# chao-ji/ldm_tf2

Measured on AMD Instinct MI355X. Metric: images/sec (256x256, 200 DDIM steps, CFG=5), higher is better.
Workload: dtype bf16

## Files before the change

### ldm_tf2_amd/csrc/gemm.hip

```cpp
#include "gemm_kernel.h"
#include "gemm3_kernel.h"

using namespace ldm_gemm_detail;

namespace {

__global__ __launch_bounds__(256) void splitk_epilogue_kernel(GemmArgs p) {
  const int nout = p.act == LDM_ACT_GEGLU ? p.N / 2 : p.N;
  const int64_t total = (int64_t)p.M * nout;
  for (int64_t idx = (int64_t)blockIdx.x * 256 + threadIdx.x; idx < total;
       idx += (int64_t)gridDim.x * 256) {
    const int m = (int)(idx / nout), c = (int)(idx - (int64_t)m * nout);
    if (p.act == LDM_ACT_GEGLU) {
      const int nv = (c >> 5) * 64 + (c & 31), ng = nv + 32;
      float a = 0.f, g = 0.f;
      for (int s = 0; s < p.split_k; ++s) {
        const float* ws = p.ws + ((int64_t)s * p.M + m) * p.N;
        a += ws[nv]; g += ws[ng];
      }
      epi_store(p, 0, m, c, epi_pre(p, m, nv, a) * gelu_erf_f(epi_pre(p, m, ng, g)));
    } else {
      float a = 0.f;
      for (int s = 0; s < p.split_k; ++s) a += p.ws[((int64_t)s * p.M + m) * p.N + c];
      epi_store(p, 0, m, c, apply_act(p.act, epi_pre(p, m, c, a)));
// ... 23 lines not shown
    const f32x4 t0 = *(const f32x4*)(src + s * slab), t1 = *(const f32x4*)(src + s * slab + 4);
#pragma unroll
    for (int e = 0; e < 4; ++e) { v[e] += t0[e]; v[4 + e] += t1[e]; }
  }
  if (p.bias) {
    const f32x4 b0 = *(const f32x4*)(p.bias + nlog), b1 = *(const f32x4*)(p.bias + nlog + 4);
#pragma unroll
    for (int e = 0; e < 4; ++e) { v[e] = v[e] * p.alpha + b0[e]; v[4 + e] = v[4 + e] * p.alpha + b1[e]; }
  } else {
#pragma unroll
    for (int e = 0; e < 8; ++e) v[e] *= p.alpha;
  }
  if (p.addend) {
    const float* ad = p.addend + (int64_t)(m / p.add_rows) * p.add_ld + nlog;
    const f32x4 a0 = *(const f32x4*)ad, a1 = *(const f32x4*)(ad + 4);
#pragma unroll
    for (int e = 0; e < 4; ++e) { v[e] += a0[e]; v[4 + e] += a1[e]; }
  }
}

__global__ __launch_bounds__(256) void splitk_epilogue_vec_kernel(GemmArgs p) {
  const bool geglu = p.act == LDM_ACT_GEGLU;
  const int nout = geglu ? p.N / 2 : p.N;
  const int pcols = nout / 8;
  const int64_t total = (int64_t)p.M * pcols;
  for (int64_t idx = (int64_t)blockIdx.x * 256 + threadIdx.x; idx < total;
       idx += (int64_t)gridDim.x * 256) {
    const int m = (int)(idx / pcols), c = (int)(idx - (int64_t)m * pcols) * 8;
    const int nlog = geglu ? (c >> 5) * 64 + (c & 31) : c;
    float v[8];
    splitk_sum8(p, m, nlog, v);
    if (geglu) {
      float g[8];
      splitk_sum8(p, m, nlog + 32, g);
#pragma unroll
      for (int e = 0; e < 8; ++e) v[e] *= gelu_erf_f(g[e]);
    } else if (p.act != LDM_ACT_NONE) {
#pragma unroll
      for (int e = 0; e < 8; ++e) v[e] = apply_act(p.act, v[e]);
    }
    const int64_t ooff = (int64_t)m * p.ldc_m + c;
    const int64_t roff = (int64_t)m * p.ldr + c;
    if (p.out_dtype == LDM_BF16) {
      if (p.residual) {
        float rr[8];
        chunk_to_f32(*(const u32x4*)((const bf16_t*)p.residual + roff), rr, bf16_t());
#pragma unroll
        for (int e = 0; e < 8; ++e) v[e] += rr[e];
      }
      *(u32x4*)((bf16_t*)p.out + ooff) = f32_to_chunk(v, bf16_t());
    } else {
      if (p.residual) {
        const f32x4 r0 = *(const f32x4*)((const float*)p.residual + roff);
        const f32x4 r1 = *(const f32x4*)((const float*)p.residual + roff + 4);
#pragma unroll
        for (int e = 0; e < 4; ++e) { v[e] += r0[e]; v[4 + e] += r1[e]; }
      }
      f32x4 o0 = {v[0], v[1], v[2], v[3]}, o1 = {v[4], v[5], v[6], v[7]};
      *(f32x4*)((float*)p.out + ooff) = o0;
      *(f32x4*)((float*)p.out + ooff + 4) = o1;
    }
  }
}

struct TileCfg { int bm, bn; };
constexpr int kNumTiles = 20;
constexpr TileCfg kTiles[kNumTiles] = {{0, 0}, {256, 128}, {128, 128}, {128, 64}, {64, 64}, {256, 128},
                                       {128, 160}, {256, 160}, {128, 320},
                                       {256, 160}, {128, 160}, {256, 128}, {128, 128},
                                       {256, 160}, {256, 128},
                                       {256, 160}, {256, 128},
                                       {64, 64}, {128, 64}, {128, 128}};
constexpr int kResident[kNumTiles] = {0, 1, 2, 3, 5, 1, 2, 1, 1, 1, 2, 1, 2, 1, 1, 1, 1, 2, 2, 1};
constexpr bool kBf16Only[kNumTiles] = {false, false, false, false, false, false, false, false, false, true, true, true, true, true, true,
                                       true, true, false, false, false};
constexpr bool is_persistent(int c) { return c == 13 || c == 14; }
constexpr bool is_halo_ring(int c) { return c == 15 || c == 16; }
bool halo_ring_ok(const ldm_gemm_params* p) {
  return p->conv && p->stride == 1 && !p->upsample && !p->no_lead_pad && p->dtype == LDM_BF16 && p->batch == 1 &&
         (p->W == 16 || p->W == 32) && 256 % p->W == 0 && p->H % (256 / p->W) == 0 && p->M % 256 == 0 &&
         p->OH == p->H && p->OW == p->W;
}

template <typename T>
void launch_mode(int cfg, const GemmArgs& a, dim3 grid, hipStream_t s) {
  if (cfg == 15 || cfg == 16) {
    if constexpr (sizeof(T) == 2) launch_cfg<T, 3>(cfg, a, grid, s);
    return;
  }
  if (!a.conv) launch_cfg<T, 0>(cfg, a, grid, s);
  else if (!a.upsample) launch_cfg<T, 1>(cfg, a, grid, s);
  else launch_cfg<T, 2>(cfg, a, grid, s);
}

inline int cdiv(int a, int b) { return (a + b - 1) / b; }

void choose(const ldm_gemm_params* p, int esize, int* cfg_out, int* split_out) {
  static const double kStepUs[kNumTiles] = {0, 0.82, 0.82, 0.75, 0.87, 0.82, 1.12, 1.18, 1.15, 1.03, 1.09, 0.97, 0.80, 1.03, 0.97, 1.0, 0.94, 0.87, 0.75, 0.82};
  static const double kOverheadSteps[kNumTiles] = {0, 8, 8, 7, 6, 8, 8, 8, 8, 8, 8, 8, 8, 4, 4, 9, 9, 6, 7, 8};
  static const int kSplits[] = {1, 2, 3, 4, 5, 6, 8, 10, 12, 16, 20, 24, 32};
#ifdef LDM_TOOLS_BUILD
  static const bool no160 = getenv("LDM_GEMM_NO160") != nullptr;
  static const bool no_t2pref = getenv("LDM_GEMM_NO_T2PREF") != nullptr;
#else
  constexpr bool no160 = false, no_t2pref = false;
#endif
  const int bke = 128 / esize;
  const int ktiles = cdiv(p->K, bke);
  const bool geglu = p->act == LDM_ACT_GEGLU;
  const double f32x = esize == 4 ? 8.0 : 1.0;
  double best = 1e30;
  int best_cfg = 2, best_split = 1;
  for (int c = 1; c < kNumTiles; ++c) {
    if (p->tile > 0 && p->tile < kNumTiles && c != p->tile) continue;
    if (c == 5 && p->tile != 5) continue;
    if (c >= 13 && p->tile != c) continue;
    if (c == 12 && p->tile != c) continue;
    if ((c == 1 || c == 7) && esize == 2 && p->tile != c) continue;
    if (c == 6 && esize == 2 && p->tile != 6) continue;
    if (kBf16Only[c] && esize != 2) continue;
    if (p->a2 && (is_persistent(c) || is_halo_ring(c)) && p->tile != c) continue;
    if (kTiles[c].bn % 160 == 0 && p->tile != c && (p->N % kTiles[c].bn != 0 || no160)) continue;
    if (p->out2 && p->n_split % kTiles[c].bn != 0) continue;
    if (geglu && c > 2 && c != 5 && c != 11 && c != 12 && c != 14 && c != 19) continue;
    const TileCfg t = kTiles[c];
    const double tiles = (double)cdiv(p->M, t.bm) * cdiv(p->N, t.bn) * p->batch;
    for (int split : kSplits) {
      if (p->split_k > 0 && split != p->split_k) continue;
      if (is_persistent(c) && split > 1) continue;
      if (split > 1 && (p->batch != 1 || ktiles / split < 4 || tiles >= 256.0 * kResident[c] ||
                        (p->split_k <= 0 && (!p->workspace || (size_t)split * p->M * p->N * 4 > p->workspace_bytes))))
        continue;
      const int kps = cdiv(ktiles, split);
      const double rounds = (double)(int64_t)((tiles * split + 256.0 * kResident[c] - 1) / (256.0 * kResident[c]));
      double us = rounds * (kps + kOverheadSteps[c]) * kStepUs[c] * f32x;
      if (!no_t2pref && c == 2 && (double)cdiv(p->M, 256) * cdiv(p->N, 128) * p->batch < 256.0) us *= 0.9;
      if (split > 1) us += 3.0 + (double)p->M * p->N * 4.0 * (split + 1) / 3.0e6;
      if (us < best) { best = us; best_cfg = c; best_split = split; }
    }
  }
  if (p->split_k > 0 && p->batch == 1) best_split = p->split_k;
  if (p->tile > 0 && p->tile < kNumTiles) best_cfg = p->tile;
  else if (best_cfg == 9 && halo_ring_ok(p) && p->N % 160 == 0 && !p->out2 && !p->ln_out && !p->a2 && ktiles / best_split >= 27)
    best_cfg = 15;
  *cfg_out = best_cfg;
  *split_out = best_split;
}

void final_plan(const ldm_gemm_params* p, int* cfg_out, int* split_out, int* kps_out) {
  const int esize = p->dtype == LDM_BF16 ? 2 : 4;
  int cfg, split;
  choose(p, esize, &cfg, &split);
  if (p->ln_out) { cfg = kLnTile; split = 1; }
  if (p->ln_cs && !is_persistent(cfg)) {
    cfg = (p->act == LDM_ACT_GEGLU || p->N % 160 != 0) ? 14 : (p->N % 128 == 0 && p->tile != 13 ? 14 : 13);
    split = 1;
  }
  if (p->out2 && !is_persistent(cfg)) split = 1;
  if (is_persistent(cfg)) split = 1;
  const int ktiles = cdiv(p->K, 128 / esize);
  int kps = cdiv(ktiles, split < 1 ? 1 : split);
  if (is_halo_ring(cfg)) kps = cdiv(kps, 9) * 9;
  split = cdiv(ktiles, kps);
  *cfg_out = cfg; *split_out = split; *kps_out = kps;
}

void build_args(const ldm_gemm_params* p, int cfg, int split, int kps, GemmArgs* out) {
  const int esize = p->dtype == LDM_BF16 ? 2 : 4;
  const int bke = 128 / esize;
  int64_t a_bytes;
  if (p->conv) a_bytes = (((int64_t)p->B * p->H * p->W - 1) * p->lda + p->Cin) * esize;
  else a_bytes = (((int64_t)p->M - 1) * p->lda + (p->K - (p->a2 ? p->Cin2 : 0))) * esize;
  const int64_t w_bytes = (int64_t)p->N * p->K * esize;
  GemmArgs a;
  memset(&a, 0, sizeof(a));
  a.a = (const char*)p->a; a.w = (const char*)p->w; a.bias = p->bias; a.addend = p->addend;
  a.residual = (const char*)p->residual; a.out = (char*)p->out; a.ws = (float*)p->workspace;
  a.lda = p->lda; a.ldr = p->ldr; a.ldc_m = p->ldc_m; a.ldc_n = p->ldc_n;
  a.stride_a = p->stride_a; a.stride_w = p->stride_w; a.stride_c = p->stride_c; a.stride_r = p->stride_r;
  a.add_ld = p->add_ld; a.M = p->M; a.N = p->N; a.K = p->K; a.batch = p->batch;
  a.a_bytes = (uint32_t)a_bytes; a.w_bytes = (uint32_t)w_bytes;
  a.add_rows = p->add_rows > 0 ? p->add_rows : 1;
  a.conv = p->conv; a.H = p->H; a.W = p->W; a.Cin = p->Cin; a.OH = p->OH; a.OW = p->OW;
  a.stride = p->stride; a.upsample = p->upsample; a.pad = p->no_lead_pad ? 0 : 1; a.act = p->act; a.out_dtype = p->out_dtype;
  a.alpha = p->alpha;
  a.ln_out = (char*)p->ln_out; a.ln_gamma = p->ln_gamma; a.ln_beta = p->ln_beta; a.ld_ln = p->ld_ln;
  a.ln_eps = p->ln_eps;
  a.out2 = (char*)p->out2; a.ld2 = p->ld2; a.stride2 = p->stride2; a.n_split = p->n_split; a.rows2 = p->rows2;
  a.kt9 = cdiv(p->K, bke);
  if (p->a2) {
    a.a2 = (const char*)p->a2; a.lda2 = p->lda2; a.kt9 = (p->K - p->Cin2) / bke;
    a.a2_bytes = (uint32_t)((((int64_t)p->M - 1) * p->lda2 + p->Cin2) * esize);
  }
  const int nout = p->act == LDM_ACT_GEGLU ? p->N / 2 : p->N;
  auto al = [](const void* q, int by) { return ((uintptr_t)q % by) == 0; };
  a.vec_epilogue =
      p->ldc_n == 1 && nout % 8 == 0 && p->ldc_m % 8 == 0 && p->stride_c % 8 == 0 && al(p->out, 16) &&
      (!p->residual || (p->ldr % 8 == 0 && p->stride_r % 8 == 0 && al(p->residual, 16))) &&
      (!p->bias || al(p->bias, 16)) &&
      (!p->addend || (al(p->addend, 16) && p->add_ld % 4 == 0));
  a.ktiles = cdiv(p->K, bke);
  a.split_k = split;
  a.ktiles_per_split = kps;
  const TileCfg t = kTiles[cfg];
  a.tiles_m = cdiv(p->M, t.bm);
  a.tiles_n = cdiv(p->N, t.bn);
  *out = a;
}

int launch_reduce(const ldm_gemm_params* p, const GemmArgs& a, hipStream_t s) {
  const int nout = p->act == LDM_ACT_GEGLU ? p->N / 2 : p->N;
  const bool vec = a.vec_epilogue && ((uintptr_t)p->workspace % 16) == 0 && p->N % 4 == 0;
  int64_t total = vec ? (int64_t)p->M * (nout / 8) : (int64_t)p->M * nout;
  int blocks = (int)((total + 255) / 256);
  if (blocks > 4096) blocks = 4096;
  if (vec) hipLaunchKernelGGL(splitk_epilogue_vec_kernel, dim3(blocks), dim3(256), 0, s, a);
  else hipLaunchKernelGGL(splitk_epilogue_kernel, dim3(blocks), dim3(256), 0, s, a);
  return ldm_launch_status("ldm_gemm(splitk epilogue)");
}

}

extern "C" int ldm_gemm_splits(const ldm_gemm_params* p) {
  if (!p || !(p->dtype == LDM_F32 || p->dtype == LDM_BF16) || p->K <= 0) return 0;
  int cfg, split, kps;
  final_plan(p, &cfg, &split, &kps);
  return split;
}

extern "C" int ldm_gemm_reduce(const ldm_gemm_params* p, void* stream) {
  LDM_CHECK_ARG(p && p->out && p->workspace, "ldm_gemm_reduce: null pointer");
  int cfg, split, kps;
  final_plan(p, &cfg, &split, &kps);
  LDM_CHECK_ARG(split > 1, "ldm_gemm_reduce: these parameters do not split K (nothing was deferred)");
  LDM_CHECK_ARG(p->workspace_bytes >= (size_t)split * p->M * p->N * 4, "ldm_gemm_reduce: workspace too small");
  GemmArgs a;
  build_args(p, cfg, split, kps, &a);
  return launch_reduce(p, a, (hipStream_t)stream);
}

extern "C" size_t ldm_gemm_workspace_bytes(const ldm_gemm_params* p) {
  if (!p) return 0;
  int cfg, split, kps;
  final_plan(p, &cfg, &split, &kps);
  return split > 1 ? (size_t)split * p->M * p->N * 4 : 0;
}

extern "C" int ldm_gemm_ln_supported(int N, int dtype) {
  return (N == kTiles[kLnTile].bn && (dtype == LDM_F32 || dtype == LDM_BF16)) ? 1 : 0;
}

extern "C" int ldm_gemm_plan(const ldm_gemm_params* p, int* tile, int* split_k) {
  LDM_CHECK_ARG(p && tile && split_k, "ldm_gemm_plan: null pointer");
  LDM_CHECK_ARG(p->dtype == LDM_F32 || p->dtype == LDM_BF16, "ldm_gemm_plan: bad dtype %d", p->dtype);
  int kps;
  final_plan(p, tile, split_k, &kps);
  return LDM_OK;
}

extern "C" int ldm_gemm(const ldm_gemm_params* p, void* stream) {
  LDM_CHECK_ARG(p && p->a && p->w && p->out, "ldm_gemm: null pointer");
  LDM_CHECK_ARG(p->dtype == LDM_F32 || p->dtype == LDM_BF16, "ldm_gemm: bad dtype %d", p->dtype);
  LDM_CHECK_ARG(p->out_dtype == LDM_F32 || p->out_dtype == LDM_BF16, "ldm_gemm: bad out_dtype");
  LDM_CHECK_ARG(p->M > 0 && p->N > 0 && p->K > 0 && p->batch > 0, "ldm_gemm: bad M/N/K/batch");
  const int esize = p->dtype == LDM_BF16 ? 2 : 4;
  const int osize = p->out_dtype == LDM_BF16 ? 2 : 4;
  const int epc = 16 / esize, bke = 8 * epc;
  LDM_CHECK_ARG(p->K % bke == 0, "ldm_gemm: K=%d must be a multiple of the K-tile (%d elements)", p->K, bke);
  LDM_CHECK_ARG(((uintptr_t)p->a % 16) == 0 && ((uintptr_t)p->w % 16) == 0,
                "ldm_gemm: a/w must be 16-byte aligned");
  LDM_CHECK_ARG(p->lda % epc == 0 && p->stride_a % epc == 0 && p->stride_w % epc == 0,
                "ldm_gemm: lda/stride_a/stride_w must be multiples of %d elements", epc);
  int64_t a_bytes;
  if (p->conv) {
    LDM_CHECK_ARG(p->Cin > 0 && p->Cin % bke == 0, "ldm_gemm(conv): Cin=%d must be a multiple of %d",
                  p->Cin, bke);
    LDM_CHECK_ARG(p->K == 9 * p->Cin + (p->a2 ? p->Cin2 : 0), "ldm_gemm(conv): K must be 9*Cin (+ Cin2 with a second operand)");
    if (p->a2) {
      LDM_CHECK_ARG(p->stride == 1 && !p->upsample && !p->no_lead_pad && p->OH == p->H && p->OW == p->W,
                    "ldm_gemm(conv): the second operand (a2) needs a stride-1, pad-1, non-upsampled convolution");
      LDM_CHECK_ARG(p->Cin2 > 0 && p->Cin2 % bke == 0 && p->lda2 % epc == 0 && p->lda2 >= p->Cin2 && ((uintptr_t)p->a2 % 16) == 0,
                    "ldm_gemm(conv): a2 needs Cin2 %% %d == 0, lda2 %% %d == 0 and 16-byte alignment", bke, epc);
      LDM_CHECK_ARG((((int64_t)p->M - 1) * p->lda2 + p->Cin2) * esize < (1ll << 31), "ldm_gemm(conv): a2 extent must be < 2 GiB");
    }
    LDM_CHECK_ARG(p->stride == 1 || p->stride == 2, "ldm_gemm(conv): stride must be 1 or 2");
    LDM_CHECK_ARG(p->B > 0 && p->H > 0 && p->W > 0 && p->OH > 0 && p->OW > 0, "ldm_gemm(conv): dims");
    LDM_CHECK_ARG(p->H < 32768 && p->W < 32768, "ldm_gemm(conv): H/W too large");
    LDM_CHECK_ARG(!(p->upsample && p->stride != 1), "ldm_gemm(conv): upsample needs stride 1");
    const int hs = p->upsample ? 2 * p->H : p->H, wsz = p->upsample ? 2 * p->W : p->W;
    LDM_CHECK_ARG(!p->no_lead_pad || p->stride == 2, "ldm_gemm(conv): no_lead_pad needs stride 2");
    const int padsum = p->no_lead_pad ? 1 : 2;
    LDM_CHECK_ARG(p->OH == (hs + padsum - 3) / p->stride + 1 && p->OW == (wsz + padsum - 3) / p->stride + 1,
                  "ldm_gemm(conv): OH/OW inconsistent with H/W/stride/upsample");
    LDM_CHECK_ARG(p->M == p->B * p->OH * p->OW, "ldm_gemm(conv): M != B*OH*OW");
    LDM_CHECK_ARG(p->batch == 1, "ldm_gemm(conv): batch must be 1");
    a_bytes = (((int64_t)p->B * p->H * p->W - 1) * p->lda + p->Cin) * esize;
  } else {
    a_bytes = (((int64_t)p->M - 1) * p->lda + p->K) * esize;
  }
  const int64_t w_bytes = (int64_t)p->N * p->K * esize;
  LDM_CHECK_ARG(a_bytes < (1ll << 31) && w_bytes < (1ll << 31),
                "ldm_gemm: operand extent must be < 2 GiB (a=%lld w=%lld bytes)", (long long)a_bytes,
                (long long)w_bytes);
  if (p->addend) LDM_CHECK_ARG(p->add_rows > 0, "ldm_gemm: add_rows must be > 0 with addend");
// ... 35 lines not shown
  if (p->act == LDM_ACT_GEGLU) LDM_CHECK_ARG(cfg <= 2 || cfg == 5 || cfg == 11 || cfg == 12 || cfg == 14 || cfg == 19, "ldm_gemm: GEGLU needs a tile whose width is a multiple of 64 (1, 2, 5, 11, 12)");
  LDM_CHECK_ARG(!kBf16Only[cfg] || esize == 2, "ldm_gemm: tile %d is bf16 only", cfg);
  LDM_CHECK_ARG(!p->a2 || (!is_persistent(cfg) && !is_halo_ring(cfg) && cfg < kNumTiles),
                "ldm_gemm: tile %d cannot take a second A operand (a2): implicit-GEMM tiles 1-12, 17-19 only", cfg);
  if (is_halo_ring(cfg))
    LDM_CHECK_ARG(halo_ring_ok(p) && p->N % kTiles[cfg].bn == 0 && !p->out2 && !p->ln_out,
                  "ldm_gemm: tile %d (halo-staged conv) needs a bf16 stride-1 3x3 convolution with W = 16 or 32, "
                  "H %% (256 / W) == 0, M %% 256 == 0 and N %% %d == 0", cfg, kTiles[cfg].bn);
  if (is_persistent(cfg)) {
    const int bn = kTiles[cfg].bn;
    auto al16 = [](const void* q) { return ((uintptr_t)q % 16) == 0; };
    const bool trans = p->out2 != nullptr;
    const bool ln = p->ln_cs != nullptr;
    const bool nsplit_out = trans && p->n_split > 0;
    if (ln)
      LDM_CHECK_ARG(!p->conv && p->bias && al16(p->ln_cs) && p->ln_eps > 0.f && !p->addend && !p->residual,
                    "ldm_gemm: ln_cs (LayerNorm fold) needs plain rows, the folded bias, ln_eps > 0 and no addend / residual");
    if (trans)
      LDM_CHECK_ARG((p->n_split == 0 || (ln && p->n_split % bn == 0 && p->n_split < p->N)) && !p->conv && (!p->bias || ln) &&
                        !p->addend && !p->residual && p->act == LDM_ACT_NONE &&
                        p->rows2 > 0 && p->rows2 % 32 == 0 && p->M % p->rows2 == 0 && p->ld2 % 8 == 0 && p->stride2 % 8 == 0 &&
                        al16(p->out2),
                    "ldm_gemm: tile %d transposed output needs n_split 0 (or, LayerNorm-folded, whole n-tiles below it), a plain "
                    "product, rows2 %% 32 == 0, ld2 / stride2 %% 8 == 0", cfg);
    LDM_CHECK_ARG(p->dtype == LDM_BF16 && p->out_dtype == LDM_BF16 && p->batch == 1 && p->ldc_n == 1 &&
                      !p->ln_out && split <= 1 && p->N % bn == 0 && ((trans && !nsplit_out) || (p->ldc_m % 8 == 0 && al16(p->out))) &&
                      (!p->residual || (p->ldr % 4 == 0 && al16(p->residual))) && (!p->bias || al16(p->bias)) &&
                      (!p->addend || (al16(p->addend) && p->add_ld % 4 == 0)),
                  "ldm_gemm: tile %d (persistent) needs bf16 in/out, batch 1, a row-major 16-byte-aligned output, "
                  "N %% %d == 0, no split-K / out2 / ln_out", cfg, bn);
    Gemm3Args g;
    memset(&g, 0, sizeof(g));
    g.a = (const char*)p->a; g.w = (const char*)p->w; g.bias = p->bias; g.addend = p->addend;
    g.residual = (const char*)p->residual; g.out = (char*)p->out;
    g.lda = p->lda; g.ldr = p->ldr; g.ldc = p->ldc_m; g.add_ld = p->add_ld;
    g.a_bytes = (uint32_t)a_bytes; g.w_bytes = (uint32_t)w_bytes;
    g.M = p->M; g.N = p->N; g.K = p->K; g.add_rows = p->add_rows > 0 ? p->add_rows : 1;
    g.conv = p->conv; g.H = p->H; g.W = p->W; g.Cin = p->Cin; g.OH = p->OH; g.OW = p->OW;
    g.stride = p->stride; g.upsample = p->upsample; g.pad = p->no_lead_pad ? 0 : 1;
    g.act = p->act;
    LDM_CHECK_ARG(p->alpha == 1.0f, "ldm_gemm: tile %d (persistent) needs alpha == 1", cfg);
#ifdef LDM_TOOLS_BUILD
    { static const int dbg = getenv("LDM_G3_DEBUG") ? atoi(getenv("LDM_G3_DEBUG")) : 0; g.dbg = dbg; }
#endif
    g.ktiles = p->K / 64;
    g.panels = cdiv(p->M, 256);
    g.ntiles = p->N / bn;
    int nsplit = p->split_k < 0 ? -p->split_k : (256 + g.panels / 2) / g.panels;
    if (nsplit < 1) nsplit = 1;
    if (nsplit > g.ntiles) nsplit = g.ntiles;
    g.tiles_per_wg = cdiv(g.ntiles, nsplit);
    g.nsplit = cdiv(g.ntiles, g.tiles_per_wg);
    if (nsplit_out) g.ntiles1 = p->n_split / bn;
    dim3 grid3((unsigned)(g.panels * g.nsplit));
    hipStream_t s3 = (hipStream_t)stream;
    g.out_t = (char*)p->out2; g.ld_t = p->ld2; g.stride_t = p->stride2; g.rows_t = p->rows2; g.n_split = p->n_split;
    g.ln_cs = p->ln_cs; g.ln_eps = p->ln_eps;
    const int epi = (trans ? (ln ? (kEpiTrans | kEpiBias | (nsplit_out ? kEpiSplit : 0)) : kEpiTrans)
                           : epi_code(p->bias != nullptr, p->addend != nullptr, p->residual != nullptr, p->act)) | (ln ? kEpiLn : 0);
    bool ok;
    if (ln) ok = launch_gemm3_ln(bn / 32, epi, g, grid3, s3);
    else if (!p->conv) ok = launch_gemm3<0>(bn / 32, epi, g, grid3, s3);
    else if (!p->upsample) ok = launch_gemm3<1>(bn / 32, epi, g, grid3, s3);
    else ok = launch_gemm3<2>(bn / 32, epi, g, grid3, s3);
    LDM_CHECK_ARG(ok, "ldm_gemm: tile %d (persistent) has no kernel for this epilogue (bias %d addend %d residual %d act %d)",
                  cfg, p->bias != nullptr, p->addend != nullptr, p->residual != nullptr, p->act);
    return ldm_launch_status("ldm_gemm(persistent)");
  }
  GemmArgs a;
  build_args(p, cfg, split, kps, &a);
  if (p->ln_out) LDM_CHECK_ARG(a.vec_epilogue, "ldm_gemm: ln_out needs the 16-byte-aligned row-major epilogue");
  if (split > 1) {
    const size_t need = (size_t)split * p->M * p->N * 4;
    if (!p->workspace || p->workspace_bytes < need) {
      ldm_set_error("ldm_gemm: split_k=%d needs %zu workspace bytes, have %zu", split, need,
                    p->workspace ? p->workspace_bytes : (size_t)0);
      return LDM_ERR_WORKSPACE;
    }
  }
  const int64_t nblk = (int64_t)a.tiles_m * a.tiles_n * (split > 1 ? split : p->batch);
  LDM_CHECK_ARG(nblk < (1ll << 31), "ldm_gemm: grid too large");
  dim3 grid((unsigned)nblk);
  hipStream_t s = (hipStream_t)stream;
  if (p->dtype == LDM_BF16) launch_mode<bf16_t>(cfg, a, grid, s);
  else launch_mode<float>(cfg, a, grid, s);
  int st = ldm_launch_status("ldm_gemm");
  if (st != LDM_OK) return st;
  if (split > 1 && !p->defer_reduce) st = launch_reduce(p, a, s);
  return st;
}
```

### ldm_tf2_amd/csrc/gemm_kernel.h

```cpp
#pragma once
#include "common.h"
#include <stdlib.h>

namespace ldm_gemm_detail {


struct GemmArgs {
  const char* a;
  const char* w;
  const float* bias;
  const float* addend;
  const char* residual;
  char* out;
  float* ws;
  int64_t lda, ldr, ldc_m, ldc_n;
  int64_t stride_a, stride_w, stride_c, stride_r;
  int64_t add_ld;
  uint32_t a_bytes, w_bytes;
  int M, N, K, batch;
  int add_rows;
  int conv, H, W, Cin, OH, OW, stride, upsample, pad;
  int act, out_dtype;
  int split_k, ktiles_per_split, ktiles;
  int tiles_m, tiles_n;
  int vec_epilogue;
  float alpha;
  char* ln_out;
  const float* ln_gamma;
  const float* ln_beta;
  int64_t ld_ln;
  float ln_eps;
  char* out2;
  int64_t ld2, stride2;
  int n_split, rows2;
  const char* a2;
  int64_t lda2;
  uint32_t a2_bytes;
  int kt9;
};

constexpr int kLnTile = 8;

constexpr uint32_t kOOB = 0x80000000u;

__device__ __forceinline__ void mma32(f32x16& acc, const u32x4& a, const u32x4& b, bf16_t) {
  acc = __builtin_amdgcn_mfma_f32_32x32x16_bf16(__builtin_bit_cast(bf16x8, a),
                                                __builtin_bit_cast(bf16x8, b), acc, 0, 0, 0);
}
__device__ __forceinline__ void mma32(f32x16& acc, const u32x4& a, const u32x4& b, float) {
#pragma unroll
  for (int j = 0; j < 4; ++j)
    acc = __builtin_amdgcn_mfma_f32_32x32x2f32(__uint_as_float(a[j]), __uint_as_float(b[j]), acc,
                                               0, 0, 0);
}

__device__ __forceinline__ uint32_t pick6(int j, uint32_t a0, uint32_t a1, uint32_t a2, uint32_t a3, uint32_t a4, uint32_t a5) {
  uint32_t v = a0;
  v = j == 1 ? a1 : v;
  v = j == 2 ? a2 : v;
  v = j == 3 ? a3 : v;
  v = j == 4 ? a4 : v;
  v = j == 5 ? a5 : v;
  return v;
}

__device__ __forceinline__ float epi_pre(const GemmArgs& p, int m, int n, float acc) {
  float v = acc * p.alpha;
  if (p.bias) v += p.bias[n];
  if (p.addend) v += p.addend[(int64_t)(m / p.add_rows) * p.add_ld + n];
  return v;
}

__device__ __forceinline__ void epi_store(const GemmArgs& p, int bz, int m, int ncol, float v) {
  const int64_t off = (int64_t)bz * p.stride_c + (int64_t)m * p.ldc_m + (int64_t)ncol * p.ldc_n;
  if (p.out_dtype == LDM_BF16) {
    if (p.residual)
      v += bf2f(((const bf16_t*)p.residual)[(int64_t)bz * p.stride_r + (int64_t)m * p.ldr + ncol]);
    ((bf16_t*)p.out)[off] = f2bf(v);
  } else {
    if (p.residual)
      v += ((const float*)p.residual)[(int64_t)bz * p.stride_r + (int64_t)m * p.ldr + ncol];
    ((float*)p.out)[off] = v;
  }
}

__device__ __forceinline__ float apply_act(int act, float v) {
  if (act == LDM_ACT_GELU) return gelu_erf_f(v);
  if (act == LDM_ACT_SILU) return silu_f(v);
  return v;
}

template <typename T, int BM, int BN, int WM, int WN, int MODE, int MF = 0, int ST = 0, int NS = 0>
__global__ __launch_bounds__(WM* WN * 64) void gemm_kernel(GemmArgs p) {
#if defined(__HIP_DEVICE_COMPILE__)
  constexpr int NW = WM * WN;
  constexpr int NT = NW * 64;
  constexpr int WTM = BM / WM, WTN = BN / WN;
  constexpr int MB = MF ? 16 : 32;
  constexpr int TM = WTM / MB, TN = WTN / MB;
  constexpr int NR = MF ? 4 : 16;
  constexpr int NIB = BN / 8;
  constexpr int LA = BM / (8 * NW), LB = (NIB + NW - 1) / NW;
  constexpr int LBF = NIB / NW;
  constexpr int NL = LA + LB;
  constexpr int ES = (int)sizeof(T);
  constexpr int EPC = 16 / ES;
  constexpr int BKE = 8 * EPC;
  constexpr bool RING = MODE == 3;
  static_assert(!RING || (MF == 1 && ST == 1 && sizeof(T) == 2 && BM == 256), "halo-staged conv: bf16 ping-pong tiles");
  constexpr int PROWS = 344;
  constexpr int PATCH = PROWS * 128;
  constexpr int LAP = (PROWS / 8 + NW - 1) / NW;
  constexpr int STAGE = RING ? BN * 128 : (BM + BN) * 128;
  constexpr int kLds = 160 * 1024;
  constexpr int NSTAGE = NS ? NS : RING ? 3 : (4 * STAGE > kLds && 3 * STAGE <= kLds && WM * WN == 8) ? 3 : 2;
  static_assert(NSTAGE >= 2 && NSTAGE <= 4 && (!NS || (!RING && !ST)), "ring depth");
  constexpr int RINGB = RING ? 2 * PATCH : 0;
  constexpr int ESPLIT = (BN % 160 == 0 && WM >= 2) ? 2 : 1;
  constexpr int EROWS = BM / ESPLIT;
  constexpr int SMEM = RINGB + NSTAGE * STAGE > EROWS * BN * 4 ? RINGB + NSTAGE * STAGE : EROWS * BN * 4;
  static_assert(SMEM <= kLds, "LDS");
  static_assert(LA >= 1 && LB >= 1 && TM >= 1 && TN >= 1 && BM % (8 * NW) == 0 && BN % 8 == 0, "tile");
  static_assert(WTM % MB == 0 && WTN % MB == 0, "wave tile must be whole MFMA blocks");
  static_assert(!MF || (ES == 2 && WTM % 16 == 0 && (WTN / 2) % 8 == 0), "16x16x32 path: bf16, swizzle-aligned wave tiles");
  static_assert(EROWS % WTM == 0, "epilogue row pass must hold whole wave tiles");
  typedef __attribute__((address_space(3))) void* lds_ptr;

  __shared__ __attribute__((aligned(16))) char smem[SMEM];

  const int tid = threadIdx.x;
  const int lane = tid & 63;
  const int wave = __builtin_amdgcn_readfirstlane(tid >> 6);
  const int wm = wave / WN, wn = wave % WN;

  const int ntile = p.tiles_m * p.tiles_n;
  int bid = blockIdx.x;
  {
    const int nwg = gridDim.x;
    const int q = nwg >> 3, r = nwg & 7, x = bid & 7;
    bid = (x < r ? x * (q + 1) : r * (q + 1) + (x - r) * q) + (bid >> 3);
  }
  const int tile_id = bid % ntile;
  const int zz = bid / ntile;
  const int tile_m = tile_id / p.tiles_n, tile_n = tile_id % p.tiles_n;
  const int split = p.split_k > 1 ? zz : 0;
  const int bz = p.split_k > 1 ? 0 : zz;
  const int m0 = tile_m * BM, n0 = tile_n * BN;

  const int kt_begin = split * p.ktiles_per_split;
  const int kt_end = min(p.ktiles, kt_begin + p.ktiles_per_split);
  const int nk = kt_end - kt_begin;

  const __amdgpu_buffer_rsrc_t rsA = __builtin_amdgcn_make_buffer_rsrc(
      const_cast<char*>(p.a) + (int64_t)bz * p.stride_a * ES, 0, p.a_bytes, 0x00020000);
  const __amdgpu_buffer_rsrc_t rsW = __builtin_amdgcn_make_buffer_rsrc(
      const_cast<char*>(p.w) + (int64_t)bz * p.stride_w * ES, 0, p.w_bytes, 0x00020000);

  int a_base[LA], a_mask[LA], a_aux[LA];
  [[maybe_unused]] int a2_base[LA];
#pragma unroll
  for (int i = 0; i < LA; ++i) {
    const int row = (i * NW + wave) * 8 + (lane >> 3);
    const int ck = (lane & 7) ^ ((row >> 1) & 7);
    const int m = m0 + row;
    a_base[i] = MODE == 0 ? (int)kOOB : 0; a_mask[i] = 0; a_aux[i] = 0;
    if constexpr (MODE <= 1) a2_base[i] = m < p.M ? (int)((int64_t)m * p.lda2 * ES) + ck * 16 : (int)kOOB;
    if (m < p.M) {
      if constexpr (MODE != 0) {
        const int ohw = p.OH * p.OW;
        const int b = m / ohw, rem = m - b * ohw;
        const int oy = rem / p.OW, ox = rem - oy * p.OW;
        const int iy0 = oy * p.stride - p.pad, ix0 = ox * p.stride - p.pad;
        const int Hs = MODE == 2 ? p.H * 2 : p.H, Ws = MODE == 2 ? p.W * 2 : p.W;
        int mask = 0;
#pragma unroll
        for (int t = 0; t < 9; ++t) {
          const int iy = iy0 + t / 3, ix = ix0 + t % 3;
          if ((unsigned)iy < (unsigned)Hs && (unsigned)ix < (unsigned)Ws) mask |= 1 << t;
        }
        a_mask[i] = mask;
        if constexpr (MODE == 2) {
          a_base[i] = (int)((int64_t)b * p.H * p.W * p.lda * ES) + ck * 16;
          a_aux[i] = (iy0 << 16) | (ix0 & 0xffff);
        } else {
          a_base[i] = (int)(((int64_t)(b * p.H + iy0) * p.W + ix0) * p.lda * ES) + ck * 16;
        }
      } else {
        a_base[i] = (int)((int64_t)m * p.lda * ES) + ck * 16;
      }
    }
  }
  int b_base[LB];
#pragma unroll
  for (int i = 0; i < LB; ++i) {
    const int row = (i * NW + wave) * 8 + (lane >> 3);
    const int ck = (lane & 7) ^ ((row >> 1) & 7);
    const int n = n0 + row;
    b_base[i] = (n < p.N && row < BN) ? (int)((int64_t)n * p.K * ES) + ck * 16 : (int)kOOB;
  }
  const bool b_last = LB == LBF || (LBF * NW + wave) < NIB;
  const int row_pitch = (int)(p.lda * ES);
  const int line_pitch = p.W * row_pitch;

  [[maybe_unused]] const __amdgpu_buffer_rsrc_t rsA2 = __builtin_amdgcn_make_buffer_rsrc(
      const_cast<char*>(MODE <= 1 && p.a2 ? p.a2 : p.a), 0, MODE <= 1 && p.a2 ? p.a2_bytes : 0u, 0x00020000);
  auto issue_tile = [&](int kt, int stage) {
    char* dA = smem + stage * STAGE + wave * 1024;
    char* dB = dA + BM * 128;
    int kb;
    if (MODE <= 1 && kt >= p.kt9) {
      const int kb2 = (kt - p.kt9) * 128;
      kb = kt * 128;
#pragma unroll
      for (int i = 0; i < LA; ++i)
        __builtin_amdgcn_raw_ptr_buffer_load_lds(rsA2, (lds_ptr)(dA + i * NW * 1024), 16,
                                                 (uint32_t)a2_base[i] + (uint32_t)kb2, 0, 0, 0);
    } else if constexpr (MODE != 0) {
      const int cc = kt / 9;
      const int tap = kt - cc * 9;
      const int cib = cc * 128;
      kb = tap * p.Cin * ES + cib;
      const int kh = tap / 3, kw = tap - kh * 3;
      if constexpr (MODE == 2) {
#pragma unroll
        for (int i = 0; i < LA; ++i) {
          const int iy = ((a_aux[i] >> 16) + kh) >> 1;
          const int ix = ((int)(short)(a_aux[i] & 0xffff) + kw) >> 1;
          const uint32_t off = (uint32_t)(a_base[i] + iy * line_pitch + ix * row_pitch + cib);
          __builtin_amdgcn_raw_ptr_buffer_load_lds(rsA, (lds_ptr)(dA + i * NW * 1024), 16,
                                                   ((a_mask[i] >> tap) & 1) ? off : kOOB, 0, 0, 0);
        }
      } else {
        const int toff = kh * line_pitch + kw * row_pitch + cib;
#pragma unroll
        for (int i = 0; i < LA; ++i) {
          const uint32_t off = (uint32_t)(a_base[i] + toff);
          __builtin_amdgcn_raw_ptr_buffer_load_lds(rsA, (lds_ptr)(dA + i * NW * 1024), 16,
                                                   ((a_mask[i] >> tap) & 1) ? off : kOOB, 0, 0, 0);
        }
      }
    } else {
      kb = kt * 128;
#pragma unroll
      for (int i = 0; i < LA; ++i)
        __builtin_amdgcn_raw_ptr_buffer_load_lds(rsA, (lds_ptr)(dA + i * NW * 1024), 16,
                                                 (uint32_t)a_base[i] + (uint32_t)kb, 0, 0, 0);
    }
#pragma unroll
    for (int i = 0; i < LBF; ++i)
      __builtin_amdgcn_raw_ptr_buffer_load_lds(rsW, (lds_ptr)(dB + i * NW * 1024), 16,
                                               (uint32_t)b_base[i] + (uint32_t)kb, 0, 0, 0);
    if constexpr (LB != LBF) {
      if (b_last)
        __builtin_amdgcn_raw_ptr_buffer_load_lds(rsW, (lds_ptr)(dB + LBF * NW * 1024), 16,
                                                 (uint32_t)b_base[LBF] + (uint32_t)kb, 0, 0, 0);
    }
  };

  static_assert(!RING || LAP == 6, "patch piece slots");
  [[maybe_unused]] uint32_t ao0 = kOOB, ao1 = kOOB, ao2 = kOOB, ao3 = kOOB, ao4 = kOOB, ao5 = kOOB;
  [[maybe_unused]] int prow0[TM];
  [[maybe_unused]] int pw = 0, prows = 0;
  if constexpr (RING) {
    const int lines = BM / p.W;
    pw = p.W + 2;
    prows = (lines + 2) * pw;
    const int tpi = p.H / lines;
    const int img = tile_m / tpi, l0 = (tile_m - img * tpi) * lines;
    auto piece_off = [&](int j) __attribute__((always_inline)) -> uint32_t {
      const int row = (j * NW + wave) * 8 + (lane >> 3);
      const int ck = (lane & 7) ^ (row & 7);
      const int line = row / pw, px = row - line * pw - 1;
      const int iy = l0 - 1 + line;
      if (row < prows && (unsigned)iy < (unsigned)p.H && (unsigned)px < (unsigned)p.W && m0 < p.M)
        return (uint32_t)((((int64_t)img * p.H + iy) * p.W + px) * p.lda * ES) + ck * 16;
      return kOOB;
    };
    ao0 = piece_off(0); ao1 = piece_off(1); ao2 = piece_off(2);
    ao3 = piece_off(3); ao4 = piece_off(4); ao5 = piece_off(5);
#pragma unroll
    for (int i = 0; i < TM; ++i) {
      const int r = wm * WTM + i * MB + (lane & 15);
      const int line = r / p.W;
      prow0[i] = line * pw + (r - line * p.W);
    }
  }
  [[maybe_unused]] auto issue_patch_piece = [&](int lc, int chunk, int j) __attribute__((always_inline)) -> int {
    if constexpr (RING) {
      if ((j * NW + wave) * 8 >= prows) return 0;
      const uint32_t off = pick6(j, ao0, ao1, ao2, ao3, ao4, ao5);
      __builtin_amdgcn_raw_ptr_buffer_load_lds(rsA, (lds_ptr)(smem + (lc & 1) * PATCH + (j * NW + wave) * 1024), 16,
                                               off + (uint32_t)chunk * 128u, 0, 0, 0);
      return 1;
    }
    return 0;
  };
  [[maybe_unused]] auto issue_w = [&](int chunk, int tap, int stage) __attribute__((always_inline)) {
    if constexpr (RING) {
      char* dB = smem + RINGB + stage * STAGE + wave * 1024;
      const uint32_t kb = (uint32_t)(tap * p.Cin * ES + chunk * 128);
#pragma unroll
      for (int i = 0; i < LBF; ++i)
        __builtin_amdgcn_raw_ptr_buffer_load_lds(rsW, (lds_ptr)(dB + i * NW * 1024), 16, (uint32_t)b_base[i] + kb, 0, 0, 0);
      if constexpr (LB != LBF) {
        if (b_last)
          __builtin_amdgcn_raw_ptr_buffer_load_lds(rsW, (lds_ptr)(dB + LBF * NW * 1024), 16, (uint32_t)b_base[LBF] + kb, 0, 0, 0);
      }
    }
  };

  typedef float AccV __attribute__((ext_vector_type(NR)));
  AccV acc[TM][TN];
#pragma unroll
  for (int i = 0; i < TM; ++i)
#pragma unroll
    for (int j = 0; j < TN; ++j)
#pragma unroll
      for (int r = 0; r < NR; ++r) acc[i][j][r] = 0.f;

  constexpr int KS = MF ? 2 : 4;
  const int lr = MF ? (lane & 15) : (lane & 31), lh = MF ? (lane >> 4) : (lane >> 5);
  const int sw = (lr >> 1) & 7;
  int offA[KS], offB[KS];
#pragma unroll
  for (int kg = 0; kg < KS; ++kg) {
    const int coff = ((MF ? (kg * 4 + lh) : (kg * 2 + lh)) ^ sw) << 4;
    offA[kg] = (wm * WTM + lr) * 128 + coff;
    offB[kg] = (RING ? 0 : BM * 128) + (wn * WTN + lr) * 128 + coff;
  }

  if constexpr (!RING) {
    if (nk > 0) issue_tile(kt_begin, 0);
    if (NSTAGE >= 3 && nk > 1) issue_tile(kt_begin + 1, 1);
    if (NSTAGE >= 4 && nk > 2) issue_tile(kt_begin + 2, 2);
  }
  u32x4 fa[KS][TM], fb[KS][TN];
  auto wait_tile = [&](int t) {
    const int ahead = min(NSTAGE - 2, nk - 1 - t);
    if (NSTAGE >= 4 && ahead == 2) {
      if (b_last) asm volatile("s_waitcnt vmcnt(%0)" ::"n"(2 * NL) : "memory");
      else asm volatile("s_waitcnt vmcnt(%0)" ::"n"(2 * (NL - 1)) : "memory");
    } else if (NSTAGE >= 3 && ahead == 1) {
      if (b_last) asm volatile("s_waitcnt vmcnt(%0)" ::"n"(NL) : "memory");
      else asm volatile("s_waitcnt vmcnt(%0)" ::"n"(NL - 1) : "memory");
    } else {
      asm volatile("s_waitcnt vmcnt(0)" ::: "memory");
    }
  };
  auto read_frags = [&](const char* cS) {
#pragma unroll
    for (int kg = 0; kg < KS; ++kg) {
#pragma unroll
      for (int i = 0; i < TM; ++i) fa[kg][i] = *(const u32x4*)(cS + offA[kg] + i * MB * 128);
#pragma unroll
      for (int j = 0; j < TN; ++j) fb[kg][j] = *(const u32x4*)(cS + offB[kg] + j * MB * 128);
    }
  };
  auto multiply = [&]() {
    __builtin_amdgcn_s_setprio(1);
#pragma unroll
    for (int kg = 0; kg < KS; ++kg) {
#pragma unroll
      for (int i = 0; i < TM; ++i)
#pragma unroll
        for (int j = 0; j < TN; ++j) {
          if constexpr (MF) {
            acc[i][j] = __builtin_amdgcn_mfma_f32_16x16x32_bf16(__builtin_bit_cast(bf16x8, fa[kg][i]),
                                                                __builtin_bit_cast(bf16x8, fb[kg][j]), acc[i][j], 0, 0, 0);
          } else {
            mma32(acc[i][j], fa[kg][i], fb[kg][j], T());
          }
        }
    }
    __builtin_amdgcn_s_setprio(0);
  };
  int st = 0;
  const bool late = ST && wave >= NW / 2;
  if constexpr (RING) {
    const int nchunks = nk / 9, c_begin = kt_begin / 9;
#pragma unroll
    for (int j = 0; j < LAP; ++j) issue_patch_piece(0, c_begin, j);
    if (nk > 0) issue_w(c_begin, 0, 0);
    if (nk > 1) issue_w(c_begin, 1, 1);
    int lc = 0, tap = 0, prev_a = 0;
    auto wait_step = [&](int s) __attribute__((always_inline)) {
      if (s + 1 < nk) {
        const int extra = prev_a + (b_last ? 1 : 0);
        if (extra == 2) asm volatile("s_waitcnt vmcnt(%0)" ::"n"(LB + 1) : "memory");
        else if (extra == 1) asm volatile("s_waitcnt vmcnt(%0)" ::"n"(LB) : "memory");
        else asm volatile("s_waitcnt vmcnt(%0)" ::"n"(LB - 1) : "memory");
      } else {
        asm volatile("s_waitcnt vmcnt(0)" ::: "memory");
      }
    };
    auto stage_next = [&](int s) __attribute__((always_inline)) {
      prev_a = 0;
      if (tap < LAP && lc + 1 < nchunks) prev_a = issue_patch_piece(lc + 1, c_begin + lc + 1, tap);
      if (s + 2 < nk) {
        int t2 = tap + 2, c2 = lc;
        if (t2 >= 9) { t2 -= 9; ++c2; }
        int s2 = st + 2;
        s2 = s2 >= 3 ? s2 - 3 : s2;
        issue_w(c_begin + c2, t2, s2);
      }
    };
    int adr[KS][TM];
    auto calc_addr = [&]() __attribute__((always_inline)) {
      const int kh = tap / 3, kw = tap - 3 * kh;
      const int shift = kh * pw + kw;
      const int pbase = (lc & 1) * PATCH;
#pragma unroll
      for (int i = 0; i < TM; ++i) {
        const int row = prow0[i] + shift;
        const int sw = row & 7;
#pragma unroll
        for (int kg = 0; kg < KS; ++kg) adr[kg][i] = pbase + row * 128 + (((kg * 4 + lh) ^ sw) << 4);
      }
    };
    calc_addr();
    auto read_ring = [&]() __attribute__((always_inline)) {
      const char* cB = smem + RINGB + st * STAGE;
#pragma unroll
      for (int kg = 0; kg < KS; ++kg) {
#pragma unroll
        for (int i = 0; i < TM; ++i) fa[kg][i] = *(const u32x4*)(smem + adr[kg][i]);
#pragma unroll
        for (int j = 0; j < TN; ++j) fb[kg][j] = *(const u32x4*)(cB + offB[kg] + j * MB * 128);
      }
    };
    auto advance = [&]() __attribute__((always_inline)) {
      st = st + 1 == 3 ? 0 : st + 1;
      if (++tap == 9) { tap = 0; ++lc; }
    };
    if (!late) {
      for (int s = 0; s < nk; ++s) {
        wait_step(s);
        __builtin_amdgcn_s_barrier();
        stage_next(s);
        read_ring();
        advance();
        calc_addr();
        multiply();
      }
    } else {
      for (int s = 0; s < nk; ++s) {
        wait_step(s);
        __builtin_amdgcn_s_barrier();
        if (s > 0) multiply();
        stage_next(s);
        read_ring();
        advance();
        calc_addr();
        asm volatile("s_waitcnt lgkmcnt(0)" ::: "memory");
        __builtin_amdgcn_sched_barrier(0);
      }
      if (nk > 0) multiply();
    }
  } else if (!late) {
    for (int t = 0; t < nk; ++t) {
      wait_tile(t);
      __builtin_amdgcn_s_barrier();
// ... 292 lines not shown
```

### ldm_tf2_amd/csrc/gemm_launch.h

```cpp
#pragma once
#include "gemm_kernel.h"

namespace ldm_gemm_detail {

template <typename T, int MODE>
void launch_cfg(int cfg, const GemmArgs& a, dim3 grid, hipStream_t s) {
  if constexpr (MODE == 3) {
    if constexpr (sizeof(T) == 2) {
      if (cfg == 15) hipLaunchKernelGGL((gemm_kernel<T, 256, 160, 4, 2, 3, 1, 1>), grid, dim3(512), 0, s, a);
      else hipLaunchKernelGGL((gemm_kernel<T, 256, 128, 4, 2, 3, 1, 1>), grid, dim3(512), 0, s, a);
    }
  } else
  switch (cfg) {
    case 1: hipLaunchKernelGGL((gemm_kernel<T, 256, 128, 4, 2, MODE>), grid, dim3(512), 0, s, a); break;
    case 2: hipLaunchKernelGGL((gemm_kernel<T, 128, 128, 2, 2, MODE>), grid, dim3(256), 0, s, a); break;
    case 3: hipLaunchKernelGGL((gemm_kernel<T, 128, 64, 2, 2, MODE>), grid, dim3(256), 0, s, a); break;
    case 5: hipLaunchKernelGGL((gemm_kernel<T, 256, 128, 2, 2, MODE>), grid, dim3(256), 0, s, a); break;
    case 6: hipLaunchKernelGGL((gemm_kernel<T, 128, 160, 4, 1, MODE>), grid, dim3(256), 0, s, a); break;
    case 7: hipLaunchKernelGGL((gemm_kernel<T, 256, 160, 8, 1, MODE>), grid, dim3(512), 0, s, a); break;
    case 8: hipLaunchKernelGGL((gemm_kernel<T, 128, 320, 4, 2, MODE>), grid, dim3(512), 0, s, a); break;
    case 9: case 10: case 11: case 12:
      if constexpr (sizeof(T) == 2) {
        if (cfg == 9) hipLaunchKernelGGL((gemm_kernel<T, 256, 160, 4, 2, MODE, 1, 1>), grid, dim3(512), 0, s, a);
        else if (cfg == 10) hipLaunchKernelGGL((gemm_kernel<T, 128, 160, 2, 2, MODE, 1>), grid, dim3(256), 0, s, a);
        else if (cfg == 11) hipLaunchKernelGGL((gemm_kernel<T, 256, 128, 4, 2, MODE, 1, 1>), grid, dim3(512), 0, s, a);
        else hipLaunchKernelGGL((gemm_kernel<T, 128, 128, 2, 2, MODE, 1>), grid, dim3(256), 0, s, a);
      }
      break;
    case 17: hipLaunchKernelGGL((gemm_kernel<T, 64, 64, 2, 2, MODE, 0, 0, 4>), grid, dim3(256), 0, s, a); break;
    case 18: hipLaunchKernelGGL((gemm_kernel<T, 128, 64, 2, 2, MODE, 0, 0, 3>), grid, dim3(256), 0, s, a); break;
    case 19: hipLaunchKernelGGL((gemm_kernel<T, 128, 128, 2, 2, MODE, 0, 0, 3>), grid, dim3(256), 0, s, a); break;
    default: hipLaunchKernelGGL((gemm_kernel<T, 64, 64, 2, 2, MODE>), grid, dim3(256), 0, s, a); break;
  }
}

}
```

Measured before the change: 9.435.

## Add multi-image halo-staged conv GEMM path for small spatial maps

Adds a new kernel mode for stride-1 3x3 convs whose feature map holds at most 64 pixels, so one 256-row tile covers several whole images. Each channel chunk is staged into LDS once and reused across the 9 taps, with per-row boundary masks that point out-of-image taps at a zero row. Weights are prefetched through a deeper ring of up to 5 stages. This removes repeated global reads of activations for the smallest UNet levels, at the cost of more LDS, extra address arithmetic per tap, and K splits forced to whole 9-tap chunks.

```diff
diff --git a/ldm_tf2_amd/csrc/gemm.hip b/ldm_tf2_amd/csrc/gemm.hip
--- a/ldm_tf2_amd/csrc/gemm.hip
+++ b/ldm_tf2_amd/csrc/gemm.hip
@@ -129,10 +129,29 @@
          p->OH == p->H && p->OW == p->W;
 }
 
+bool halo_multi_ok(const ldm_gemm_params* p) {
+  const int hw = p->H * p->W;
+  return p->conv && p->stride == 1 && !p->upsample && !p->no_lead_pad && p->dtype == LDM_BF16 && p->batch == 1 &&
+         !p->a2 && !p->out2 && !p->ln_out && hw > 0 && hw <= 64 && 256 % hw == 0 && p->M % 256 == 0 &&
+         p->OH == p->H && p->OW == p->W;
+}
+#ifdef LDM_TOOLS_BUILD
+bool g_halo_multi_off = false;
+#else
+constexpr bool g_halo_multi_off = false;
+#endif
+bool halo_multi(const ldm_gemm_params* p, int cfg) {
+  return (cfg == 9 || cfg == 11) && !g_halo_multi_off && halo_multi_ok(p) && p->N % kTiles[cfg].bn == 0;
+}
+
 template <typename T>
-void launch_mode(int cfg, const GemmArgs& a, dim3 grid, hipStream_t s) {
+void launch_mode(int cfg, bool hm, const GemmArgs& a, dim3 grid, hipStream_t s) {
   if (cfg == 15 || cfg == 16) {
     if constexpr (sizeof(T) == 2) launch_cfg<T, 3>(cfg, a, grid, s);
+    return;
+  }
+  if (hm) {
+    if constexpr (sizeof(T) == 2) launch_cfg<T, 4>(cfg, a, grid, s);
     return;
   }
   if (!a.conv) launch_cfg<T, 0>(cfg, a, grid, s);
@@ -207,7 +226,7 @@
   if (is_persistent(cfg)) split = 1;
   const int ktiles = cdiv(p->K, 128 / esize);
   int kps = cdiv(ktiles, split < 1 ? 1 : split);
-  if (is_halo_ring(cfg)) kps = cdiv(kps, 9) * 9;
+  if (is_halo_ring(cfg) || halo_multi(p, cfg)) kps = cdiv(kps, 9) * 9;
   split = cdiv(ktiles, kps);
   *cfg_out = cfg; *split_out = split; *kps_out = kps;
 }
@@ -267,6 +286,10 @@
 }
 
 }
+
+#ifdef LDM_TOOLS_BUILD
+extern "C" void ldm_gemm_set_halo_multi(int on) { g_halo_multi_off = !on; }
+#endif
 
 extern "C" int ldm_gemm_splits(const ldm_gemm_params* p) {
   if (!p || !(p->dtype == LDM_F32 || p->dtype == LDM_BF16) || p->K <= 0) return 0;
@@ -468,8 +491,10 @@
   LDM_CHECK_ARG(nblk < (1ll << 31), "ldm_gemm: grid too large");
   dim3 grid((unsigned)nblk);
   hipStream_t s = (hipStream_t)stream;
-  if (p->dtype == LDM_BF16) launch_mode<bf16_t>(cfg, a, grid, s);
-  else launch_mode<float>(cfg, a, grid, s);
+  const bool hm = halo_multi(p, cfg);
+  if (hm) LDM_CHECK_ARG(kps % 9 == 0 && a.ktiles % 9 == 0, "ldm_gemm: multi-image halo form needs whole channel chunks per split");
+  if (p->dtype == LDM_BF16) launch_mode<bf16_t>(cfg, hm, a, grid, s);
+  else launch_mode<float>(cfg, false, a, grid, s);
   int st = ldm_launch_status("ldm_gemm");
   if (st != LDM_OK) return st;
   if (split > 1 && !p->defer_reduce) st = launch_reduce(p, a, s);
diff --git a/ldm_tf2_amd/csrc/gemm_inst_bf16_m4.hip b/ldm_tf2_amd/csrc/gemm_inst_bf16_m4.hip
--- /dev/null
+++ b/ldm_tf2_amd/csrc/gemm_inst_bf16_m4.hip
@@ -0,0 +1,4 @@
+#include "gemm_launch.h"
+namespace ldm_gemm_detail {
+template void launch_cfg<bf16_t, 4>(int, const GemmArgs&, dim3, hipStream_t);
+}
diff --git a/ldm_tf2_amd/csrc/gemm_kernel.h b/ldm_tf2_amd/csrc/gemm_kernel.h
--- a/ldm_tf2_amd/csrc/gemm_kernel.h
+++ b/ldm_tf2_amd/csrc/gemm_kernel.h
@@ -64,6 +64,16 @@
   return v;
 }
 
+__device__ __forceinline__ void vm_wait(int n) {
+#define LDM_VMW(k) case k: asm volatile("s_waitcnt vmcnt(%0)" ::"n"(k) : "memory"); break;
+  switch (n) {
+    LDM_VMW(1) LDM_VMW(2) LDM_VMW(3) LDM_VMW(4) LDM_VMW(5) LDM_VMW(6) LDM_VMW(7) LDM_VMW(8)
+    LDM_VMW(9) LDM_VMW(10) LDM_VMW(11) LDM_VMW(12) LDM_VMW(13) LDM_VMW(14) LDM_VMW(15)
+    default: asm volatile("s_waitcnt vmcnt(0)" ::: "memory"); break;
+  }
+#undef LDM_VMW
+}
+
 __device__ __forceinline__ float epi_pre(const GemmArgs& p, int m, int n, float acc) {
   float v = acc * p.alpha;
   if (p.bias) v += p.bias[n];
@@ -106,16 +116,19 @@
   constexpr int ES = (int)sizeof(T);
   constexpr int EPC = 16 / ES;
   constexpr int BKE = 8 * EPC;
-  constexpr bool RING = MODE == 3;
+  constexpr bool HM = MODE == 4;
+  constexpr bool RING = MODE == 3 || HM;
   static_assert(!RING || (MF == 1 && ST == 1 && sizeof(T) == 2 && BM == 256), "halo-staged conv: bf16 ping-pong tiles");
-  constexpr int PROWS = 344;
+  constexpr int PROWS = HM ? BM : 344;
   constexpr int PATCH = PROWS * 128;
   constexpr int LAP = (PROWS / 8 + NW - 1) / NW;
   constexpr int STAGE = RING ? BN * 128 : (BM + BN) * 128;
   constexpr int kLds = 160 * 1024;
-  constexpr int NSTAGE = NS ? NS : RING ? 3 : (4 * STAGE > kLds && 3 * STAGE <= kLds && WM * WN == 8) ? 3 : 2;
-  static_assert(NSTAGE >= 2 && NSTAGE <= 4 && (!NS || (!RING && !ST)), "ring depth");
-  constexpr int RINGB = RING ? 2 * PATCH : 0;
+  constexpr int ZROW = 2 * PATCH;
+  constexpr int RINGB = RING ? 2 * PATCH + (HM ? 128 : 0) : 0;
+  constexpr int HMST = (kLds - RINGB) / STAGE > 5 ? 5 : (kLds - RINGB) / STAGE;
+  constexpr int NSTAGE = NS ? NS : HM ? HMST : RING ? 3 : (4 * STAGE > kLds && 3 * STAGE <= kLds && WM * WN == 8) ? 3 : 2;
+  static_assert(NSTAGE >= 2 && NSTAGE <= (HM ? 5 : 4) && (!NS || (!RING && !ST)), "ring depth");
   constexpr int ESPLIT = (BN % 160 == 0 && WM >= 2) ? 2 : 1;
   constexpr int EROWS = BM / ESPLIT;
   constexpr int SMEM = RINGB + NSTAGE * STAGE > EROWS * BN * 4 ? RINGB + NSTAGE * STAGE : EROWS * BN * 4;
@@ -257,11 +270,34 @@
     }
   };
 
-  static_assert(!RING || LAP == 6, "patch piece slots");
+  static_assert(!RING || LAP == (HM ? 4 : 6), "patch piece slots");
   [[maybe_unused]] uint32_t ao0 = kOOB, ao1 = kOOB, ao2 = kOOB, ao3 = kOOB, ao4 = kOOB, ao5 = kOOB;
   [[maybe_unused]] int prow0[TM];
+  [[maybe_unused]] int hmask[TM];
   [[maybe_unused]] int pw = 0, prows = 0;
-  if constexpr (RING) {
+  if constexpr (HM) {
+    auto piece_off = [&](int j) __attribute__((always_inline)) -> uint32_t {
+      const int row = (j * NW + wave) * 8 + (lane >> 3);
+      const int ck = (lane & 7) ^ (row & 7);
+      return (uint32_t)((int64_t)(m0 + row) * p.lda * ES) + ck * 16;
+    };
+    ao0 = piece_off(0); ao1 = piece_off(1); ao2 = piece_off(2); ao3 = piece_off(3);
+    pw = p.W;
+    const int hw = p.H * p.W;
+#pragma unroll
+    for (int i = 0; i < TM; ++i) {
+      const int r = wm * WTM + i * MB + (lane & 15);
+      const int rem = r % hw, y = rem / p.W, x = rem - y * p.W;
+      int mask = 0;
+#pragma unroll
+      for (int t = 0; t < 9; ++t) {
+        const int iy = y + t / 3 - 1, ix = x + t % 3 - 1;
+        if ((unsigned)iy < (unsigned)p.H && (unsigned)ix < (unsigned)p.W) mask |= 1 << t;
+      }
+      prow0[i] = r;
+      hmask[i] = mask;
+    }
+  } else if constexpr (RING) {
     const int lines = BM / p.W;
     pw = p.W + 2;
     prows = (lines + 2) * pw;
@@ -286,7 +322,12 @@
     }
   }
   [[maybe_unused]] auto issue_patch_piece = [&](int lc, int chunk, int j) __attribute__((always_inline)) -> int {
-    if constexpr (RING) {
+    if constexpr (HM) {
+      const uint32_t off = j == 0 ? ao0 : j == 1 ? ao1 : j == 2 ? ao2 : ao3;
+      __builtin_amdgcn_raw_ptr_buffer_load_lds(rsA, (lds_ptr)(smem + (lc & 1) * PATCH + (j * NW + wave) * 1024), 16,
+                                               off + (uint32_t)chunk * 128u, 0, 0, 0);
+      return 1;
+    } else if constexpr (RING) {
       if ((j * NW + wave) * 8 >= prows) return 0;
       const uint32_t off = pick6(j, ao0, ao1, ao2, ao3, ao4, ao5);
       __builtin_amdgcn_raw_ptr_buffer_load_lds(rsA, (lds_ptr)(smem + (lc & 1) * PATCH + (j * NW + wave) * 1024), 16,
@@ -376,7 +417,91 @@
   };
   int st = 0;
   const bool late = ST && wave >= NW / 2;
-  if constexpr (RING) {
+  if constexpr (HM) {
+    constexpr int D = NSTAGE - 1;
+    static_assert(D >= 2 && D <= 9, "prefetch distance");
+    const int nchunks = nk / 9, c_begin = kt_begin / 9;
+    if (wave == 0 && lane < 8) {
+      *(u32x4*)(smem + ZROW + lane * 16) = u32x4{0u, 0u, 0u, 0u};
+      asm volatile("s_waitcnt lgkmcnt(0)" ::: "memory");
+    }
+#pragma unroll
+    for (int j = 0; j < LAP; ++j) issue_patch_piece(0, c_begin, j);
+#pragma unroll
+    for (int d = 0; d < D; ++d)
+      if (d < nk) issue_w(c_begin + d / 9, d % 9, d);
+    int lc = 0, tap = 0;
+    auto wait_step = [&](int s) __attribute__((always_inline)) {
+      const int ahead = min(D - 1, nk - 1 - s);
+      const int extra = (tap >= 1 && tap < D && lc + 1 < nchunks) ? LAP : 0;
+      vm_wait(ahead * (b_last ? LB : LBF) + extra);
+    };
+    auto stage_next = [&](int s) __attribute__((always_inline)) {
+      if (tap == 0 && lc + 1 < nchunks) {
+#pragma unroll
+        for (int j = 0; j < LAP; ++j) issue_patch_piece(lc + 1, c_begin + lc + 1, j);
+      }
+      if (s + D < nk) {
+        const int k2 = s + D, c2 = k2 / 9;
+        int s2 = st + D;
+        s2 = s2 >= NSTAGE ? s2 - NSTAGE : s2;
+        issue_w(c_begin + c2, k2 - 9 * c2, s2);
+      }
+    };
+    int adr[KS][TM];
+    auto calc_addr = [&]() __attribute__((always_inline)) {
+      const int kh = tap / 3, kw = tap - 3 * kh;
+      const int shift = (kh - 1) * pw + (kw - 1);
+      const int pbase = (lc & 1) * PATCH;
+#pragma unroll
+      for (int i = 0; i < TM; ++i) {
+        const int row = prow0[i] + shift;
+        const int base = ((hmask[i] >> tap) & 1) ? pbase + row * 128 : ZROW;
+        const int sw = row & 7;
+#pragma unroll
+        for (int kg = 0; kg < KS; ++kg) adr[kg][i] = base + (((kg * 4 + lh) ^ sw) << 4);
+      }
+    };
+    calc_addr();
+    auto read_ring = [&]() __attribute__((always_inline)) {
+      const char* cB = smem + RINGB + st * STAGE;
+#pragma unroll
+      for (int kg = 0; kg < KS; ++kg) {
+#pragma unroll
+        for (int i = 0; i < TM; ++i) fa[kg][i] = *(const u32x4*)(smem + adr[kg][i]);
+#pragma unroll
+        for (int j = 0; j < TN; ++j) fb[kg][j] = *(const u32x4*)(cB + offB[kg] + j * MB * 128);
+      }
+    };
+    auto advance = [&]() __attribute__((always_inline)) {
+      st = st + 1 == NSTAGE ? 0 : st + 1;
+      if (++tap == 9) { tap = 0; ++lc; }
+    };
+    if (!late) {
+      for (int s = 0; s < nk; ++s) {
+        wait_step(s);
+        __builtin_amdgcn_s_barrier();
+        stage_next(s);
+        read_ring();
+        advance();
+        calc_addr();
+        multiply();
+      }
+    } else {
+      for (int s = 0; s < nk; ++s) {
+        wait_step(s);
+        __builtin_amdgcn_s_barrier();
+        if (s > 0) multiply();
+        stage_next(s);
+        read_ring();
+        advance();
+        calc_addr();
+        asm volatile("s_waitcnt lgkmcnt(0)" ::: "memory");
+        __builtin_amdgcn_sched_barrier(0);
+      }
+      if (nk > 0) multiply();
+    }
+  } else if constexpr (RING) {
     const int nchunks = nk / 9, c_begin = kt_begin / 9;
 #pragma unroll
     for (int j = 0; j < LAP; ++j) issue_patch_piece(0, c_begin, j);
diff --git a/ldm_tf2_amd/csrc/gemm_launch.h b/ldm_tf2_amd/csrc/gemm_launch.h
--- a/ldm_tf2_amd/csrc/gemm_launch.h
+++ b/ldm_tf2_amd/csrc/gemm_launch.h
@@ -9,6 +9,11 @@
     if constexpr (sizeof(T) == 2) {
       if (cfg == 15) hipLaunchKernelGGL((gemm_kernel<T, 256, 160, 4, 2, 3, 1, 1>), grid, dim3(512), 0, s, a);
       else hipLaunchKernelGGL((gemm_kernel<T, 256, 128, 4, 2, 3, 1, 1>), grid, dim3(512), 0, s, a);
+    }
+  } else if constexpr (MODE == 4) {
+    if constexpr (sizeof(T) == 2) {
+      if (cfg == 9) hipLaunchKernelGGL((gemm_kernel<T, 256, 160, 4, 2, 4, 1, 1>), grid, dim3(512), 0, s, a);
+      else hipLaunchKernelGGL((gemm_kernel<T, 256, 128, 4, 2, 4, 1, 1>), grid, dim3(512), 0, s, a);
     }
   } else
   switch (cfg) {
```

Result: no change. 9.457 (median of 6 runs) (+0.2%).
